# sailab-code/GNN_tf_2.x

Measured on AMD Instinct MI355X. Metric: node-state-updates/sec (nodes x iters / s), 1M-node synthetic graph, higher is better.
Workload: dtype f32; 1 GPU; synthetic randomGraph-recipe graph, N=1000000 nodes, E=9999690 arcs, state_dim=64, net_state 135->128->128->64 selu+BN, net_output 67->2 softmax+BN, max_iter=30, threshold=0 (all iterations run); the loop-invariant label aggregates (GNN.py:259, :263; 0.2 ms) are kept between Loops until the labels change, see cold_aggregates_ms_per_step; parallelism=single GPU, tile_form=one wave per 32-node tile (k_fused)

## Files before the change

gnn_tf_2.x_amd/csrc/gnn_build.hip:

```cpp
#include <hipcub/hipcub.hpp>
#include <string.h>

#include <algorithm>
#include <chrono>
#include <new>
#include <vector>

#include "gnn_common.h"
#include "gnn_fused.h"

namespace {

inline unsigned cdiv(int64_t a, int64_t b) { return (unsigned)((a + b - 1) / b); }

__global__ void k_keys(int64_t e, const int32_t *src, const int32_t *dst, unsigned long long *key, int32_t *id, int32_t *indeg)
{
    const int64_t a = (int64_t)blockIdx.x * blockDim.x + threadIdx.x;
    if (a >= e) return;
    key[a] = ((unsigned long long)(uint32_t)dst[a] << 32) | (uint32_t)src[a];
    id[a] = (int32_t)a;
    atomicAdd(indeg + dst[a], 1);
}

__global__ void k_values(int64_t e, const int32_t *dst, const int32_t *indeg, int mode, float *w)
// ... 217 lines not shown
                };
                for (int r = start[g]; r < start[g + 1]; ++r) {
                    if (ip[r + 1] == ip[r]) put(GNN_GP_NOROW | GNN_GP_ROW_END | (uint32_t)r, 0.0f);
                    for (int32_t e = ip[r]; e < ip[r + 1]; ++e) {
                        if (adj_src[e] < 0 || adj_src[e] >= (1 << 23))
                            return gnn_fail(GNN_ERR_UNSUPPORTED, "adj_src[%d]=%d does not fit a gather-program source word", e, adj_src[e]);
                        put((uint32_t)adj_src[e] << 8 | (e + 1 == ip[r + 1] ? GNN_GP_ROW_END : 0u) | (uint32_t)r, adj_w[e]);
                    }
                }
                while (s < 16 * nb) put(GNN_GP_NOROW, 0.0f);
            }
        }
        batch += nb;
    }
    *n_batches = batch;
    return GNN_OK;
}

int gnn_gather_program_ensure(const gnn_graph *g)
{
    gnn_graph_shared *sh = g->sh;
    if (sh->gp_tried) return GNN_OK;
    sh->gp_tried = true;
    const int64_t tiles = g->n_rows / 32;
    if (tiles == 0) return GNN_OK;
    int dev_before = -1;
    if (hipGetDevice(&dev_before) != hipSuccess || hipSetDevice(g->device) != hipSuccess) { (void)hipGetLastError(); return GNN_OK; }
    const auto t0 = std::chrono::steady_clock::now();
    int32_t *d_hdr = nullptr, *d_ent = nullptr;
    int64_t batches = 0;
    bool ok = false;
    try {
        std::vector<int32_t> indptr((size_t)tiles * 32 + 1), hdr((size_t)tiles * 2), src, ent;
        std::vector<float> w;
        ok = hipMemcpy(indptr.data(), sh->indptr, sizeof(int32_t) * indptr.size(), hipMemcpyDeviceToHost) == hipSuccess;
        const size_t E = ok ? (size_t)indptr.back() : 0;
        src.resize(E); w.resize(E);
        ok = ok && (E == 0 || (hipMemcpy(src.data(), sh->adj_src, sizeof(int32_t) * E, hipMemcpyDeviceToHost) == hipSuccess &&
                               hipMemcpy(w.data(), sh->adj_w, sizeof(float) * E, hipMemcpyDeviceToHost) == hipSuccess));
        for (size_t e = 0; ok && e < E; ++e) ok = src[e] >= 0 && src[e] < (1 << 23);
        ok = ok && gnn_gather_program_build(tiles * 32, indptr.data(), src.data(), w.data(), hdr.data(), nullptr, &batches) == GNN_OK;
        if (ok) {
            ent.resize((size_t)batches * 128);
            ok = gnn_gather_program_build(tiles * 32, indptr.data(), src.data(), w.data(), nullptr, ent.data(), &batches) == GNN_OK;
        }
        ok = ok && gnn_dev_malloc((void **)&d_hdr, sizeof(int32_t) * hdr.size()) == hipSuccess &&
             gnn_dev_malloc((void **)&d_ent, sizeof(int32_t) * ent.size()) == hipSuccess &&
             hipMemcpy(d_hdr, hdr.data(), sizeof(int32_t) * hdr.size(), hipMemcpyHostToDevice) == hipSuccess &&
             hipMemcpy(d_ent, ent.data(), sizeof(int32_t) * ent.size(), hipMemcpyHostToDevice) == hipSuccess;
    } catch (const std::bad_alloc &) { ok = false; }
    if (ok) {
        sh->gp_hdr = d_hdr; sh->gp_ent = d_ent; sh->gp_tiles = tiles; sh->gp_batches = batches;
        sh->gp_build_ms = std::chrono::duration<float, std::milli>(std::chrono::steady_clock::now() - t0).count();
    } else {
        (void)hipFree(d_hdr); (void)hipFree(d_ent);
        (void)hipGetLastError();
    }
    (void)hipSetDevice(dev_before);
    return GNN_OK;
}

extern "C" int gnn_graph_gather_program_info(const gnn_graph *g, int64_t *tiles, int64_t *batches, int64_t *bytes, float *build_ms)
{
    ARGCHK(g, "graph is NULL");
    const gnn_graph_shared *sh = g->sh;
    const bool have = sh->gp_ent != nullptr;
    if (tiles) *tiles = have ? sh->gp_tiles : 0;
    if (batches) *batches = have ? sh->gp_batches : 0;
    if (bytes) *bytes = have ? sh->gp_tiles * 8 + sh->gp_batches * 512 : 0;
    if (build_ms) *build_ms = have ? sh->gp_build_ms : 0.0f;
    return GNN_OK;
}
```

gnn_tf_2.x_amd/csrc/gnn_common.h:

```cpp
#pragma once
#include <hip/hip_runtime.h>
#include <stdint.h>
#include <string>
#include <vector>

#include "gnn_hip.h"
#include "gnn_fused.h"

int gnn_fail(int code, const char *fmt, ...);

hipError_t gnn_dev_malloc(void **p, size_t bytes);
bool gnn_poison_enabled();

inline hipError_t gnn_raise_dynamic_lds(const void *const *kernels, int n, size_t bytes, bool (&raised)[64])
{
    int dev = 0;
    hipError_t e = hipGetDevice(&dev);
    if (e != hipSuccess) return e;
    const bool listed = dev >= 0 && dev < 64;
    if (listed && raised[dev]) return hipSuccess;
    for (int i = 0; i < n && e == hipSuccess; ++i) e = hipFuncSetAttribute(kernels[i], hipFuncAttributeMaxDynamicSharedMemorySize, (int)bytes);
    if (listed && e == hipSuccess) raised[dev] = true;
    return e;
}
// ... 109 lines not shown
    const int c0 = __hip_atomic_load(w, __ATOMIC_RELAXED, __HIP_MEMORY_SCOPE_AGENT);
    const int c1 = __hip_atomic_load(w + 1, __ATOMIC_RELAXED, __HIP_MEMORY_SCOPE_AGENT);
    const int c2 = __hip_atomic_load(w + 2, __ATOMIC_RELAXED, __HIP_MEMORY_SCOPE_AGENT);
    if (moved && c0 == 0) atomicOr(w, 1);
    if (robust && c1 == 0) atomicOr(w + 1, 1);
    if (border && c2 == 0) atomicOr(w + 2, 1);
}

struct gnn_graph_shared {
    int refs = 1;
    int32_t *indptr = nullptr, *adj_src = nullptr, *masked_rows = nullptr;
    float *adj_w = nullptr, *arc_w = nullptr, *arc_labels = nullptr;
    uint8_t *mask = nullptr;
    int max_degree = 0;
    int32_t *src_indptr = nullptr, *src_dst = nullptr;
    float *src_w = nullptr;
    int32_t *arc_id = nullptr;
    float *arc_labels_orig = nullptr;
    int32_t *full_indptr = nullptr, *full_src = nullptr;
    float *full_w = nullptr;
    int64_t full_rows = 0;
    int32_t *gp_hdr = nullptr, *gp_ent = nullptr;
    int64_t gp_tiles = 0, gp_batches = 0;
    bool gp_tried = false;
    float gp_build_ms = 0.0f;
};

struct gnn_graph {
    int device = 0;
    int64_t N = 0, N_global = 0, row_begin = 0, own_off = 0, n_rows = 0, E = 0, n_masked = 0;
    int NL = 0, AL = 0;
    int halo_world = 0, halo_rank = 0;
    int64_t halo_block = 0, halo_count = 0;
    int32_t *halo_send = nullptr;
    bool halo_send_owned = true;
    int64_t nodes_rows = 0;
    gnn_graph_shared *sh = nullptr;
    float *nodes = nullptr;
    int base_NL = 0;
    float *arc_labels_own = nullptr, *arc_labels_orig_own = nullptr;
    int base_AL = 0;
    uint64_t label_version = 1;
    hipEvent_t ready = nullptr;
};

inline const float *gnn_graph_arc_labels(const gnn_graph *g) { return g->arc_labels_own ? g->arc_labels_own : g->sh->arc_labels; }
// ... 152 lines not shown
```

gnn_tf_2.x_amd/csrc/gnn_fused.h:

```cpp
#pragma once
#include <hip/hip_runtime.h>
#include <stdint.h>

constexpr int GNN_FUSED_MAXL = 3;
constexpr int GNN_FUSED_WAVES = 8;
constexpr int GNN_FUSED_THREADS = 64 * GNN_FUSED_WAVES;
#define GNN_F16_EX 4
#define GNN_F16_LIMIT 65504.0f
#define GNN_GP_ROW_MASK 31u
#define GNN_GP_ROW_END 32u
#define GNN_GP_NOROW 0xfffffe00u
constexpr int GNN_ACTL_FROM_ARGS = -1;

struct GnnFusedArgs {
    int64_t n_rows, row_begin;
    const int32_t *indptr, *adj_src;
    const float *adj_w;
    const float *inv;
    const float *state_cur;
    float *state_nxt;
    int64_t state_bytes;
    int Ds, NLc, AL, IW, in_s, c_aggs, KP, lpr, lpr_log2, vec, kk0;
    const float *Wp[GNN_FUSED_MAXL];
    const float *bias[GNN_FUSED_MAXL];
    const float *bn_scale, *bn_shift;
    float thr;
    const int *gate;
    int *flag_out;
    int world;
    int certify;
    int *tile_ctr;
    int wstride;
    int stagger;
    const int *Ws[GNN_FUSED_MAXL];
    int chunks0;
    int pieces;
    float bsc[GNN_FUSED_MAXL], usc[GNN_FUSED_MAXL];
    const int *Ws_base;
    int ws_bytes, ws_off[GNN_FUSED_MAXL];
    int tile_base;
    int full_tiles;
    int variant;
    const float *agg_in;
    const int32_t *gp_hdr, *gp_ent;
    int gp_tiles;
    int threads;
    int single_ticket;
    unsigned long long *stamps;
    int lds_floats;
    int act_last;
};

struct GnnSmallCtl {
    float *state0, *state1;
    const float *init;
    int *kfinal;
    int *flags;
    int *host_result;
    float *xs;
    int DP;
    int rnd;
    const float *Wraw[GNN_FUSED_MAXL];
    int din[GNN_FUSED_MAXL], dout[GNN_FUSED_MAXL];
    int KP16;
    int *zero_words;
    int n_words;
    int max_iter;
    float *out;
// ... 88 lines not shown
```

gnn_tf_2.x_amd/csrc/gnn_fused.hip:

```cpp
#include <stdio.h>
#include <stdlib.h>
#include <string.h>

#include <algorithm>
#include <cmath>
#include <vector>

#include "gnn_engine.h"
#include "gnn_fused.h"

namespace {

constexpr int MAXL = GNN_FUSED_MAXL;
constexpr int K_GROUP = 12;
constexpr int K_SLACK = 8;

constexpr int GNN_FUSED_VARIANT_DEFAULT = 1;
constexpr int GNN_FUSED_SPREAD_DEFAULT = 8;
constexpr int GNN_FUSED_SPREAD_SMALL_DEFAULT = 6;
#ifndef GNN_GATHER_FORM_DEFAULT
#define GNN_GATHER_FORM_DEFAULT 2
#endif
constexpr int S_SLACK = 2;

// ... 380 lines not shown
    static const int stagger_env = getenv("GNN_FUSED_STAGGER") ? atoi(getenv("GNN_FUSED_STAGGER")) : GNN_FUSED_SPREAD_DEFAULT;
    stagger_rounds = stagger_env;
#endif
    a.stagger = n_tiles >= (size_t)4 * GNN_FUSED_WAVES * grid ? stagger_rounds : (n_tiles > (size_t)GNN_FUSED_WAVES * grid ? GNN_FUSED_SPREAD_SMALL_DEFAULT : 0);
#ifdef GNN_DIAG
    static const int stagger_small = getenv("GNN_FUSED_STAGGER_SMALL") ? atoi(getenv("GNN_FUSED_STAGGER_SMALL")) : 0;
    const bool small_grid = n_tiles > (size_t)GNN_FUSED_WAVES * grid && n_tiles < (size_t)4 * GNN_FUSED_WAVES * grid;
    if (small_grid && stagger_small > 0) { a.stagger = stagger_small; a.variant |= 4; }
    static const int spread_small = getenv("GNN_FUSED_SPREAD_SMALL") ? atoi(getenv("GNN_FUSED_SPREAD_SMALL")) : -1;
    if (small_grid && spread_small >= 0) a.stagger = spread_small;
#endif
    a.single_ticket = n_tiles <= (size_t)GNN_FUSED_WAVES * grid ? 1 : 0;
    f.grid = grid;
    f.lds = lds_bytes(p);
    if (f.kernel == GNN_BODY_PAIR) {
        const int64_t n_tiles64 = (int64_t)n_tiles;
        a.KP = pair_xs(p);
        a.full_tiles = 1;
        f.grid = (unsigned)std::min<int64_t>((int64_t)n_cu, (n_tiles64 + 3) / 4);
        a.stagger = n_tiles64 >= (int64_t)4 * 4 * f.grid ? stagger_rounds : (n_tiles64 > (int64_t)4 * f.grid ? GNN_FUSED_SPREAD_SMALL_DEFAULT : 0);
        f.lds = pair_lds_bytes(p);
    } else if (f.kernel == GNN_BODY_FULL_TILE) {
        a.full_tiles = 1;
        if (f.program) { a.gp_hdr = g->sh->gp_hdr; a.gp_ent = g->sh->gp_ent; a.gp_tiles = (int)g->sh->gp_tiles; }
    }
    a.lds_floats = gnn_poison_enabled() ? (int)(f.lds / sizeof(float)) : 0;
}

static int decide_persistent(gnn_loop *l, LoopForm &f, const SmallForm &sf)
{
    const gnn_graph *g = l->g;
    const FusedPlan &p = f.plan;
    GnnFusedArgs &a = f.args;
    fill_args(l, p, false, a);
    a.state_cur = l->state[0];
    a.state_nxt = l->state[1] + (size_t)l->own_off * l->Ds;
    GnnSmallCtl &c = f.ctl;
    c.state0 = l->state[0]; c.state1 = l->state[1];
    c.init = l->D ? l->state_init : g->nodes + (size_t)g->own_off * g->NL;
    c.kfinal = l->kfinal_dev;
    c.host_result = l->kfinal_host;
    bool tile16 = sf.tile == 16;
    f.small_wide = sf.wide;
    if (tile16) f.s0 = sf.steps; else f.kk_small = sf.steps;
#ifdef GNN_DIAG
    static const int tile_env = getenv("GNN_SMALL_TILE") ? atoi(getenv("GNN_SMALL_TILE")) : 0;
    if (tile_env == 32 && !sf.wide) {
// ... 53 lines not shown
    a.lds_floats = gnn_poison_enabled() ? (int)(f.lds / sizeof(float)) : 0;
    return GNN_OK;
}

int gnn_loop_decide_form(gnn_loop *l)
{
    LoopForm &f = l->form;
    f = LoopForm{};
    if (l->impl_req < 1) return GNN_OK;
    HIPCHK(hipSetDevice(l->device));
    if (!gnn_fused_supported(l, f.plan)) return GNN_OK;
    if (l->device < 0 || l->device >= 64) return gnn_fail(GNN_ERR_ARG, "device %d out of range", l->device);
    const gnn_graph *g = l->g;
    const FusedPlan &p = f.plan;
    const int n_cu = device_cus(l->device);
    const int64_t n_tiles = (g->n_rows + 31) / 32;
    f.split = l->impl_req == 2;
    f.pieces = l->pieces == 2 ? 2 : 3;
    const bool pair = f.split && !l->slice_mode && pair_covers(p, l->Ds) && pair_lds_bytes(p) <= 160 * 1024 &&
                      (l->tile_form ? l->tile_form == 2 : n_tiles <= (int64_t)4 * n_cu);
    f.kernel = pair ? GNN_BODY_PAIR : (l->Ds == 64 && p.NTL == 2 ? GNN_BODY_FULL_TILE : GNN_BODY_GENERIC);
    if (f.kernel == GNN_BODY_FULL_TILE && !l->slice_mode && (l->gather_form ? l->gather_form : GNN_GATHER_FORM_DEFAULT) == 2 &&
        gnn_gather_program_ensure(g) == GNN_OK)
        f.program = g->sh->gp_ent != nullptr;
    const SmallForm sf = small_form(l->st, p, g->n_rows);
    const bool persistent = l->world == 1 && !l->small_disabled && !l->profiling && sf.tile != 0;
    f.path = persistent ? GNN_PATH_PERSISTENT : GNN_PATH_BODIES;
    if (!l->inv) HIPCHK(gnn_dev_malloc((void **)&l->inv, inv_floats(l) * sizeof(float)));
    if (persistent) return decide_persistent(l, f, sf);
    decide_bodies(l, f, n_cu);
    return GNN_OK;
}

static bool launch_body(const LoopForm &f, const GnnFusedArgs &a, hipStream_t st)
{
    const FusedPlan &p = f.plan;
    if (p.act_last != p.act) {
        if (f.kernel == GNN_BODY_PAIR || p.layers < 2) return false;
        if (f.split) return p.layers == 2 ? gnn_fused_launch_ms2(p.act, p.NT, p.NTL, a, f.grid, f.lds, st) : gnn_fused_launch_ms3(p.act, p.NT, p.NTL, a, f.grid, f.lds, st);
        return p.layers == 2 ? gnn_fused_launch_ml2(p.act, p.NT, p.NTL, a, f.grid, f.lds, st) : gnn_fused_launch_ml3(p.act, p.NT, p.NTL, a, f.grid, f.lds, st);
    }
    if (f.kernel == GNN_BODY_PAIR)
        return p.layers == 2 ? gnn_fused_launch_p2(p.act, a, f.grid, f.lds, st) : gnn_fused_launch_p3(p.act, a, f.grid, f.lds, st);
    if (f.split) {
        if (p.layers == 1) return gnn_fused_launch_s1(p.act, p.NT, p.NTL, a, f.grid, f.lds, st);
        if (p.layers == 2) return gnn_fused_launch_s2(p.act, p.NT, p.NTL, a, f.grid, f.lds, st);
        return gnn_fused_launch_s3(p.act, p.NT, p.NTL, a, f.grid, f.lds, st);
// ... 86 lines not shown
```

gnn_tf_2.x_amd/csrc/gnn_fused_kernel.h:

```cpp
#pragma once
#include <utility>

#include "gnn_common.h"
#include "gnn_fused.h"

typedef float f32x16 __attribute__((ext_vector_type(16)));

namespace gnn_fused_dev {

#define GNN_GLOBAL __attribute__((address_space(1)))
template <class T>
__device__ __forceinline__ const GNN_GLOBAL T *gptr(const T *p) { return (const GNN_GLOBAL T *)p; }
template <class T>
__device__ __forceinline__ GNN_GLOBAL T *gptr_w(T *p) { return (GNN_GLOBAL T *)p; }
typedef float v4f __attribute__((ext_vector_type(4)));
typedef float v2f __attribute__((ext_vector_type(2)));
typedef int v4i_ __attribute__((ext_vector_type(4)));
__device__ __forceinline__ v4f gload4(const float *p) { return *(const GNN_GLOBAL v4f *)p; }
#ifndef GNN_STORE_AUX
#define GNN_STORE_AUX 2
#endif
__device__ __forceinline__ void gstore_row4(float *base, int64_t off, v4f v)
{
#if GNN_STORE_AUX == 0
// ... 504 lines not shown
        GNN_S0_LOAD(wa, xa, c + 1)
        GNN_S0_MFMA(wb, pb, xa, pa, false, c + 1 < n_chunks)
        GNN_S0_LOAD(wb, xb, c + 2)
        if (c + 1 < n_chunks) GNN_S0_MFMA(wa, pa, xb, pb, false, c + 2 < n_chunks)
    }
#undef GNN_S0_LOAD
#undef GNN_S0_MFMA
}

template <int NO, bool AL16>
__device__ __forceinline__ void layer0_split(const float *xr, __amdgpu_buffer_rsrc_t wrs, int voff, int soff, int n_chunks, f32x16 (&acc)[NO],
                                             const float *bias_lds, int half)
{
    float mx = 0.0f;
    layer0_split<NO, AL16, 3>(xr, wrs, voff, soff, n_chunks, acc, bias_lds, half, mx);
}

template <int NI, int NO, int ACT, int PC = 3>
__device__ __forceinline__ void layer_split_from_regs(f32x16 (&hin)[NI], const float *bias_lds, int half, f32x16 (&acc)[NO],
                                                      __amdgpu_buffer_rsrc_t wrs, int voff, int soff, float us, float &mx)
{
    using TM = SplitTerms<PC>;
    constexpr int TPU = NO >= 2 ? 2 : 1, UPC = NO / TPU, CH = 2 * NI, U = CH * UPC;
    constexpr int DEPTH = (NI + NO >= 8) ? 1 : 3;
    constexpr int NM = TM::N * NO, NTASK = 12;
    v4i w[U][TPU][PC];
    int bp[2][PC][4];
    WStream ws(soff);
#define GNN_S1_LOAD(UU)                                                                             \
    _Pragma("unroll") for (int t = 0; t < TPU; ++t)                                                 \
        _Pragma("unroll") for (int pc = 0; pc < PC; ++pc) w[UU][t][pc] = ws.next(wrs, voff);
#define GNN_S1_H(C, I) hin[(C) >> 1][8 * ((C) & 1) + (I)]
#define GNN_S1_E(C, I)                                                                              \
    if constexpr (ACT == GNN_ACT_SELU) {                                                            \
        constexpr float AL2_ = 1.6732632423543772f * 1.44269504088896341f;                          \
        const float v_ = PC == 2 ? GNN_S1_H(C, I) * us : GNN_S1_H(C, I);                            \
        GNN_S1_H(C, I) = v_ > 0.0f ? v_ : __builtin_fmaf(__builtin_amdgcn_exp2f(v_), AL2_, -AL2_);  \
    } else GNN_S1_H(C, I) = act_fast<ACT>(PC == 2 ? GNN_S1_H(C, I) * us : GNN_S1_H(C, I));
#define GNN_S1_S(C, J, DST)                                                                         \
    if constexpr (PC == 2) { float mz_ = 0.0f; split_pair_f16(GNN_S1_H(C, 2 * (J)), GNN_S1_H(C, 2 * (J) + 1), DST[0][J], DST[1][J], mz_); }   \
    else split_pair(GNN_S1_H(C, 2 * (J)), GNN_S1_H(C, 2 * (J) + 1), DST[0][J], DST[1][J], DST[PC - 1][J]);
#pragma unroll
    for (int u = 0; u < DEPTH && u < U; ++u) { GNN_S1_LOAD(u) }
    {
#pragma unroll
        for (int i = 0; i < 8; ++i) { GNN_S1_E(0, i) }
#pragma unroll
// ... 319 lines not shown
    if (t & GNN_GP_ROW_END) {
        float *xr = xo + __umul24(t & GNN_GP_ROW_MASK, (unsigned)KP);
        if constexpr (AL16) *reinterpret_cast<v4f *>(xr) = v4f{acc01.x, acc01.y, acc23.x, acc23.y};
        else { xr[0] = acc01.x; xr[1] = acc01.y; xr[2] = acc23.x; xr[3] = acc23.y; }
        acc01 = v2f{0.f, 0.f}; acc23 = v2f{0.f, 0.f};
    }
}
template <bool AL16, int GB, int... J>
__device__ __forceinline__ void prog_batch(int words, float my_w, __amdgpu_buffer_rsrc_t rsrc, int voff0, float (&w)[GB], v4f (&x)[GB],
                                           std::integer_sequence<int, J...>)
{
    ((w[J] = row_bcast_f<J>(my_w),
      x[J] = __builtin_bit_cast(v4f, __builtin_amdgcn_raw_buffer_load_b128(rsrc, (row_bcast_i<J>(words) & ~0xff) | voff0, 0, 0))), ...);
}
template <bool AL16, int GB, int... J>
__device__ __forceinline__ void prog_consume_all(int words, const float (&w)[GB], const v4f (&x)[GB], v2f &acc01, v2f &acc23, float *xo, int KP,
                                                 std::integer_sequence<int, J...>)
{
    (prog_consume<AL16, J>(words, w[J], x[J], acc01, acc23, xo, KP), ...);
}
typedef int v2i __attribute__((ext_vector_type(2)));
__device__ __forceinline__ v2i prog_header_request(const GnnFusedArgs &a, int tile)
{
    v2i h = {0, 0};
    if (tile < a.gp_tiles) h = *reinterpret_cast<const GNN_GLOBAL v2i *>(gptr(a.gp_hdr) + 2 * (int64_t)tile);
    return h;
}
__device__ __forceinline__ v2i prog_entry(const GnnFusedArgs &a, int b, int lane)
{
    return *reinterpret_cast<const GNN_GLOBAL v2i *>(gptr(a.gp_ent) + ((int64_t)b * 64 + lane) * 2);
}
template <bool AL16>
__device__ __forceinline__ void load_tile_prog64(const GnnFusedArgs &a, float *X, int64_t i0, int lane, int KP, int c_aggs, int first, int nb, v2i ent)
{
    constexpr int GB = 16;
    const int gl = lane & 15;
    TileOwn64<AL16> own;
    own.request(a, i0, lane);
    v2f acc01 = {0.f, 0.f}, acc23 = {0.f, 0.f};
    const __amdgpu_buffer_rsrc_t rsrc = __builtin_amdgcn_make_buffer_rsrc(const_cast<float *>(a.state_cur), 0, (int)a.state_bytes, 0x00020000);
    const int voff0 = gl * 16;
    float *xo = X + c_aggs + gl * 4;
    for (int b = 0; b < nb; ++b) {
        float w[GB];
        v4f x[GB];
        const int words = ent.x;
        prog_batch<AL16, GB>(words, __int_as_float(ent.y), rsrc, voff0, w, x, std::make_integer_sequence<int, GB>{});
        if (b + 1 < nb) ent = prog_entry(a, first + b + 1, lane);
        prog_consume_all<AL16, GB>(words, w, x, acc01, acc23, xo, KP, std::make_integer_sequence<int, GB>{});
    }
    own.write(a, X, i0, lane, KP, c_aggs);
}

template <bool AL16>
__device__ __forceinline__ void load_tile_given64(const GnnFusedArgs &a, float *X, int64_t i0, int lane, int KP, int c_aggs)
{
    constexpr int Ds = 64;
    v4f own[8], agg[8];
    {
        const float *src = a.state_cur + (a.row_begin + i0) * Ds + lane * 4;
        const float *sag = a.agg_in + i0 * Ds + lane * 4;
#pragma unroll
        for (int u = 0; u < 8; ++u) {
            own[u] = gload4(src + u * 256);
            agg[u] = gload4(sag + u * 256);
        }
    }
    float lab[4];
    const int IW = a.IW, nlab = 32 * IW;
    {
        const float *src = a.inv + i0 * IW;
#pragma unroll
        for (int u = 0; u < 4; ++u) lab[u] = (lane + 64 * u < nlab) ? gload1(src + lane + 64 * u) : 0.0f;
    }
#pragma unroll
    for (int u = 0; u < 8; ++u) {
// ... 69 lines not shown
        for (int u = 0; u < 16; ++u) {
            const float d = half ? o[u] : (nw[u] - o[u]);
            const float dd = d * d;
            s_ = s_ + dd;
        }
    }
    const float root = sqrtf(s_);
    const float nrm = shfl_f(root, (lane & 31) + 32);
    const float rhs = a.thr * nrm;
    const int moved = (half == 0) && (root > rhs);
    if (__any(moved) && lane == 0) gnn_flag_raise(a.flag_out);
    float *dst = a.state_nxt + i0 * Ds + lane;
    const float *xs = X + c_aggs + lane;
#pragma unroll
    for (int i = 0; i < 32; i += 8) {
        float v[8];
#pragma unroll
        for (int u = 0; u < 8; ++u) v[u] = xs[(i + u) * KP];
#pragma unroll
        for (int u = 0; u < 8; ++u) gstore_row1(dst + (i + u) * Ds, v[u]);
    }
}

__device__ __forceinline__ void finish_fast64_aligned(const GnnFusedArgs &a, float *X, f32x16 (&out)[2], int64_t i0, int lane, int KP, int c_aggs,
                                                      const GnnFlagPeek &peek)
{
    const int half = lane >> 5;
    float *xrow = X + (lane & 31) * KP;
    float d2 = 0.0f, o2 = 0.0f;
#pragma unroll
    for (int jt = 0; jt < 2; ++jt)
#pragma unroll
        for (int q = 0; q < 4; ++q) {
            const int f0 = 32 * jt + 8 * q + 4 * half;
            const v4f o = *reinterpret_cast<const v4f *>(xrow + f0);
            const v4f nw = {out[jt][4 * q], out[jt][4 * q + 1], out[jt][4 * q + 2], out[jt][4 * q + 3]};
            *reinterpret_cast<v4f *>(xrow + c_aggs + f0) = nw;
            const v4f d = nw - o;
            d2 = __builtin_fmaf(d.x, d.x, d2); d2 = __builtin_fmaf(d.y, d.y, d2); d2 = __builtin_fmaf(d.z, d.z, d2); d2 = __builtin_fmaf(d.w, d.w, d2);
            o2 = __builtin_fmaf(o.x, o.x, o2); o2 = __builtin_fmaf(o.y, o.y, o2); o2 = __builtin_fmaf(o.z, o.z, o2); o2 = __builtin_fmaf(o.w, o.w, o2);
        }
    d2 = d2 + shfl_f(d2, lane ^ 32);
    o2 = o2 + shfl_f(o2, lane ^ 32);
    const float root = sqrtf(d2), nrm = sqrtf(o2);
    {
        const float rhs = a.thr * nrm, band = GNN_BAND_ABS * nrm + GNN_BAND_REL * rhs;
        const bool am = __any(root > rhs), ar = __any(root > rhs + band), ab = __any(gnn_gate_borderline(root, rhs, band));
        if (lane == 0) gnn_flag_raise_peeked(a.flag_out, peek, am, ar, ab);
    }
    __builtin_amdgcn_fence(__ATOMIC_ACQ_REL, "wavefront");
    const int64_t dst = i0 * 64 + lane * 4;
    const float *xs = X + (lane >> 4) * KP + c_aggs + (lane & 15) * 4;
    v4f v[8];
#pragma unroll
    for (int u = 0; u < 8; ++u) v[u] = *reinterpret_cast<const v4f *>(xs + 4 * u * KP);
#pragma unroll
    for (int u = 0; u < 8; ++u) gstore_row4(a.state_nxt, dst + 256 * u, v[u]);
}

__device__ __forceinline__ void check_store_fast64_partial(const GnnFusedArgs &a, float *X, int64_t i0, int lane, int KP, int c_aggs, int nvalid)
{
    constexpr int Ds = 64;
    const int half = lane >> 5;
    const float *xo = X + (lane & 31) * KP, *xn = xo + c_aggs;
    float s_ = 0.0f;
#pragma unroll
    for (int f = 0; f < Ds; f += 16) {
        float o[16], nw[16];
#pragma unroll
        for (int u = 0; u < 16; ++u) { o[u] = xo[f + u]; nw[u] = xn[f + u]; }
// ... 102 lines not shown
    int tile = w_launch + a.tile_base, next_tile = w_launch + W_launch + a.tile_base;
    int ip_first_raw = 0;
    v2i hdr_first_raw = {0, 0};
    if constexpr (PROG) hdr_first_raw = prog_header_request(a, tile);
    else ip_first_raw = tile_rowptr_request(a, tile, lane);
    float *ep = lds + (size_t)GNN_FUSED_WAVES * 32 * KP + 32 + GNN_FUSED_WAVES * 36;
    for (int t = threadIdx.x; t < 3 * 32 * NTL; t += blockDim.x) {
        const int which = t / (32 * NTL), f = t - which * 32 * NTL;
        ep[t] = which == 0 ? a.bias[LAYERS - 1][f] * (SPLIT ? a.bsc[LAYERS - 1] : 1.0f) : (a.bn_scale ? (which == 1 ? a.bn_scale[f] : a.bn_shift[f]) : 0.0f);
    }
    float *hb = ep + 3 * 32 * NTL;
    if constexpr (SPLIT && LAYERS > 1)
        for (int t = threadIdx.x; t < (LAYERS - 1) * 32 * NT; t += blockDim.x)
            hb[t] = a.bias[t / (32 * NT)][t % (32 * NT)] * (ACT == GNN_ACT_SELU ? 1.44269504088896341f : 1.0f) * a.bsc[t / (32 * NT)];
    __syncthreads();
    if (a.stagger > 0) {
        int rounds = 0;
        if (a.variant & 4) rounds = wave >= GNN_FUSED_WAVES / 2 ? a.stagger : 0;
        else rounds = (int)((((unsigned)blockIdx.x * GNN_FUSED_WAVES + (unsigned)wave) * 0x9E3779B1u) >> 16) % (unsigned)(a.stagger + 1);
        for (int i = 0; i < rounds; ++i) __builtin_amdgcn_s_sleep(127);
    }
    int ip_cur = 0, src_cur = 0;
    float w_cur = 0.0f;
    int hdr_first = 0, hdr_nb = 0;
    v2i ent_cur = {0, 0};
    if constexpr (PROG) {
        hdr_first = __builtin_amdgcn_readfirstlane(hdr_first_raw.x); hdr_nb = __builtin_amdgcn_readfirstlane(hdr_first_raw.y);
        if (hdr_nb > 0) ent_cur = prog_entry(a, hdr_first, lane);
    } else {
        ip_cur = tile_rowptr_clamp(a, tile, lane, ip_first_raw);
        if (FULL || Ds == 64) tile_first_ids(a, ip_cur, lane, src_cur, w_cur);
    }
    if constexpr (FULL) zero_pad_columns(a, X, lane, KP);
  for (;;) {
    const int64_t i0 = (int64_t)tile * 32;
    if (i0 >= a.n_rows) break;
    const int nvalid = (int)((a0.n_rows - i0) < 32 ? (a0.n_rows - i0) : 32);
    GnnFusedArgs a = a0;
    asm volatile("" : "+s"(a.Wp[0]), "+s"(a.Wp[1]), "+s"(a.Wp[2]), "+s"(a.bias[0]), "+s"(a.bias[1]), "+s"(a.bias[2]));
    asm volatile("" : "+s"(a.bn_scale), "+s"(a.bn_shift), "+s"(a.state_cur), "+s"(a.state_nxt), "+s"(a.inv), "+s"(a.adj_src), "+s"(a.adj_w));
#ifndef GNN_DIAG
#define GNN_STAMP(slot) do { } while (0)
#else
    unsigned long long *stamp = a.stamps ? a.stamps + ((size_t)tile << 3) : nullptr;
#define GNN_STAMP(slot)                                                                      \
    do {                                                                                     \
        if (stamp) {                                                                         \
            __builtin_amdgcn_sched_barrier(0);                                               \
            const unsigned long long t_ = __builtin_amdgcn_s_memtime();                      \
            if (lane == 0) stamp[slot] = t_;                                                 \
            __builtin_amdgcn_sched_barrier(0);                                               \
        }                                                                                    \
    } while (0)
#endif
    GNN_STAMP(0);

    int *ipt = reinterpret_cast<int *>(lds + (size_t)GNN_FUSED_WAVES * 32 * KP + 32) + wave * 36;
    int ip_next_raw = 0;
    v2i hdr_next_raw = {0, 0};
    if constexpr (PROG) hdr_next_raw = prog_header_request(a, next_tile);
    else {
        if (lane <= 32) ipt[lane] = ip_cur;
        ip_next_raw = tile_rowptr_request(a, next_tile, lane);
    }
    const bool fast64 = FULL || ((Ds == 64) && (nvalid == 32) && !a.agg_in);
    if (a.variant & 1) __builtin_amdgcn_s_setprio(3);
    if constexpr (FULL && GIVEN) load_tile_given64<SPLIT>(a, X, i0, lane, KP, c_aggs);
    else if constexpr (PROG) {
        if (hdr_nb > 0) load_tile_prog64<SPLIT>(a, X, i0, lane, KP, c_aggs, hdr_first, hdr_nb, ent_cur);
        else {
            const int ip = tile_rowptr_clamp(a, tile, lane, tile_rowptr_request(a, tile, lane));
            if (lane <= 32) ipt[lane] = ip;
            tile_first_ids(a, ip, lane, src_cur, w_cur);
            load_tile_fast64<SPLIT, true>(a, X, ipt, i0, lane, KP, c_aggs, src_cur, w_cur);
        }
    }
    else if constexpr (FULL) load_tile_fast64<SPLIT, true>(a, X, ipt, i0, lane, KP, c_aggs, src_cur, w_cur);
    else {
        if (fast64) load_tile_fast64<SPLIT>(a, X, ipt, i0, lane, KP, c_aggs, src_cur, w_cur);
        else load_tile_generic(a, X, ipt, i0, lane, nvalid, KP, c_aggs);
    }
    if (a.variant & 1) __builtin_amdgcn_s_setprio(0);
    __builtin_amdgcn_fence(__ATOMIC_ACQ_REL, "wavefront");
    GNN_STAMP(2);

    const int half = lane >> 5;
    const float *xb = X + (lane & 31) * KP + half;
    f32x16 out[NTL];
    float mx = 0.0f;
    if constexpr (SPLIT) {
        const __amdgpu_buffer_rsrc_t wrs = __builtin_amdgcn_make_buffer_rsrc(const_cast<int *>(a.Ws_base), 0, a.ws_bytes, 0x00020000);
        const int wv = lane * 16;
        const float *xr = X + (lane & 31) * KP + 8 * half;
        if constexpr (LAYERS == 1) {
            layer0_split<NTL, false, PC>(xr, wrs, wv, a.ws_off[0], a.chunks0, out, ep, half, mx);
        } else {
            f32x16 h1[NT];
            if constexpr (FULL) layer0_split<NT, true, PC>(xr, wrs, wv, a.ws_off[0], a.chunks0, h1, hb, half, mx);
            else {
// ... 14 lines not shown
        }
    } else if constexpr (LAYERS == 1) {
        zero_acc<NTL>(out);
        layer_from_lds<NTL>(xb, a.Wp[0] + (size_t)lane * NTL, a.kk0, out, a.wstride);
    } else {
        f32x16 h1[NT];
        zero_acc<NT>(h1);
        layer_from_lds<NT>(xb, a.Wp[0] + (size_t)lane * NT, a.kk0, h1, a.wstride);
        GNN_STAMP(3);
        GNN_STAMP(4);
        if constexpr (LAYERS == 2) {
            zero_acc<NTL>(out);
            layer_from_regs<NT, NTL, ACT>(h1, a.bias[0], half, out, a.Wp[1] + (size_t)lane * NTL, a.wstride);
        } else {
            f32x16 h2[NT];
            zero_acc<NT>(h2);
            layer_from_regs<NT, NT, ACT>(h1, a.bias[0], half, h2, a.Wp[1] + (size_t)lane * NT, a.wstride);
            zero_acc<NTL>(out);
            layer_from_regs<NT, NTL, ACT>(h2, a.bias[1], half, out, a.Wp[2] + (size_t)lane * NTL, a.wstride);
        }
    }
    __builtin_amdgcn_fence(__ATOMIC_ACQ_REL, "wavefront");
    GNN_STAMP(5);
    int next2_tile = 0x3fffffff;
    if (third_round) {
        if (lane == 0) next2_tile = atomicAdd(a0.tile_ctr, 1) + 2 * W_launch;
    }
    int ip_next = 0, src_next = 0;
    float w_next = 0.0f;
    int hdr_first_next = 0, hdr_nb_next = 0;
    v2i ent_next = {0, 0};
    if constexpr (PROG) {
        hdr_first_next = __builtin_amdgcn_readfirstlane(hdr_next_raw.x); hdr_nb_next = __builtin_amdgcn_readfirstlane(hdr_next_raw.y);
        if (hdr_nb_next > 0) ent_next = prog_entry(a, hdr_first_next, lane);
    } else {
        ip_next = tile_rowptr_clamp(a, next_tile, lane, ip_next_raw);
        if (FULL || Ds == 64) tile_first_ids(a, ip_next, lane, src_next, w_next);
    }
    if constexpr (SPLIT && PC == 2) gnn_flag_raise_range(a.flag_out, mx);
    GnnFlagPeek peek = {0, 0, 0};
    if (SPLIT && NTL == 2 && lane == 0) peek = gnn_flag_peek(a.flag_out);
    bool finished = false;
    if constexpr (SPLIT && NTL == 2) {
        if (fast64) {
#pragma unroll
            for (int jt = 0; jt < NTL; ++jt) {
                if (a.bn_scale) tile_epilogue_last<ACTL, true, true, true, true>(a.act_last, out[jt], ep, ep + 32 * NTL, ep + 64 * NTL, jt, half, 1 << 30, a.usc[LAYERS - 1]);
                else tile_epilogue_last<ACTL, false, true, true, true>(a.act_last, out[jt], ep, nullptr, nullptr, jt, half, 1 << 30, a.usc[LAYERS - 1]);
            }
            GNN_STAMP(6);
            if (nvalid == 32) finish_fast64_aligned(a, X, out, i0, lane, KP, c_aggs, peek);
            else finish_fast64_partial(a, X, out, i0, lane, KP, c_aggs, nvalid);
            finished = true;
        }
    }
    if (!(FULL && SPLIT && NTL == 2) && !finished) {
#pragma unroll
        for (int jt = 0; jt < NTL; ++jt) {
            const float us = SPLIT ? a.usc[LAYERS - 1] : 1.0f;
            if (a.bn_scale) tile_epilogue_last<ACTL, true, SPLIT, true, SPLIT>(a.act_last, out[jt], ep, ep + 32 * NTL, ep + 64 * NTL, jt, half, 1 << 30, us);
            else tile_epilogue_last<ACTL, false, SPLIT, true, SPLIT>(a.act_last, out[jt], ep, nullptr, nullptr, jt, half, 1 << 30, us);
            float *x = X + (lane & 31) * KP + c_aggs;
#pragma unroll
            for (int r = 0; r < 16; ++r) {
                const int f = 32 * jt + (r & 3) + 8 * (r >> 2) + 4 * half;
                if (f < Ds) x[f] = out[jt][r];
            }
        }
        __builtin_amdgcn_fence(__ATOMIC_ACQ_REL, "wavefront");
        GNN_STAMP(6);
        if constexpr (FULL) {
            if (nvalid == 32) check_store_fast64(a, X, i0, lane, KP, c_aggs);
            else check_store_fast64_partial(a, X, i0, lane, KP, c_aggs, nvalid);
        } else {
            if (fast64) check_store_fast64(a, X, i0, lane, KP, c_aggs);
            else check_store_generic(a, X, i0, lane, nvalid, KP, c_aggs);
        }
    }
    GNN_STAMP(7);
#undef GNN_STAMP
    __builtin_amdgcn_fence(__ATOMIC_ACQ_REL, "wavefront");
    tile = next_tile;
    next_tile = __builtin_amdgcn_readfirstlane(next2_tile) + a0.tile_base;
    ip_cur = ip_next; src_cur = src_next; w_cur = w_next;
    hdr_first = hdr_first_next; hdr_nb = hdr_nb_next; ent_cur = ent_next;
  }
}

template <int LAYERS, int NT, int NTL, int ACT, bool SPLIT, int ACTL, bool FULL, bool GIVEN = false, int PC = 3, bool PROG = false>
inline void launch_one_pc(const GnnFusedArgs &a, unsigned grid, size_t lds_bytes, hipStream_t st)
{
    if constexpr (FULL && !GIVEN && !PROG) {
        if (a.gp_tiles > 0) { launch_one_pc<LAYERS, NT, NTL, ACT, SPLIT, ACTL, FULL, GIVEN, PC, true>(a, grid, lds_bytes, st); return; }
    }
    static bool lds_raised[64] = {false};
    (void)gnn_raise_dynamic_lds(reinterpret_cast<const void *>(&k_fused<LAYERS, NT, NTL, ACT, SPLIT, FULL, GIVEN, PC, PROG, ACTL>), 160 * 1024, lds_raised);
    hipLaunchKernelGGL((k_fused<LAYERS, NT, NTL, ACT, SPLIT, FULL, GIVEN, PC, PROG, ACTL>), grid, a.threads ? a.threads : GNN_FUSED_THREADS, lds_bytes, st, a);
}
template <int LAYERS, int NT, int NTL, int ACT, bool SPLIT, int ACTL, bool FULL, bool GIVEN = false>
inline void launch_one(const GnnFusedArgs &a, unsigned grid, size_t lds_bytes, hipStream_t st)
{
    if (SPLIT && a.pieces == 2) launch_one_pc<LAYERS, NT, NTL, ACT, SPLIT, ACTL, FULL, GIVEN, 2>(a, grid, lds_bytes, st);
    else launch_one_pc<LAYERS, NT, NTL, ACT, SPLIT, ACTL, FULL, GIVEN, 3>(a, grid, lds_bytes, st);
}

template <int LAYERS, int NT, int NTL, int ACT, bool SPLIT, int ACTL>
// ... 56 lines not shown
```

Measured before the change: 1.763 billion node-state-updates/s.

## Prefetch first gather-program batch of next tile during epilogue; cover partial last tile

Issues the buffer loads for the next tile's first gather batch, along with its second entry, before the current tile's epilogue and store, so neighbour-row fetch latency overlaps with compute. The gather program now also covers the trailing partial tile through extra header fields, which removes the CSR fallback path inside the program kernel. It adds register pressure from 16 prefetched v4f values held across the epilogue, reorders the flag raise and the tile-counter atomic, and adds a depth knob for the wide split path.

```diff
diff --git a/gnn_tf_2.x_amd/csrc/gnn_build.hip b/gnn_tf_2.x_amd/csrc/gnn_build.hip
--- a/gnn_tf_2.x_amd/csrc/gnn_build.hip
+++ b/gnn_tf_2.x_amd/csrc/gnn_build.hip
@@ -263,27 +263,33 @@
     gnn_graph_shared *sh = g->sh;
     if (sh->gp_tried) return GNN_OK;
     sh->gp_tried = true;
-    const int64_t tiles = g->n_rows / 32;
+    const int64_t tiles = g->n_rows / 32, rem = g->n_rows % 32;
     if (tiles == 0) return GNN_OK;
     int dev_before = -1;
     if (hipGetDevice(&dev_before) != hipSuccess || hipSetDevice(g->device) != hipSuccess) { (void)hipGetLastError(); return GNN_OK; }
     const auto t0 = std::chrono::steady_clock::now();
     int32_t *d_hdr = nullptr, *d_ent = nullptr;
-    int64_t batches = 0;
+    int64_t batches = 0, last_batches = 0;
+    int32_t last_hdr[2] = {0, 0};
     bool ok = false;
     try {
-        std::vector<int32_t> indptr((size_t)tiles * 32 + 1), hdr((size_t)tiles * 2), src, ent;
+        std::vector<int32_t> indptr((size_t)g->n_rows + 1), hdr((size_t)tiles * 2), src, ent;
         std::vector<float> w;
         ok = hipMemcpy(indptr.data(), sh->indptr, sizeof(int32_t) * indptr.size(), hipMemcpyDeviceToHost) == hipSuccess;
         const size_t E = ok ? (size_t)indptr.back() : 0;
+        if (rem) indptr.resize((size_t)(tiles + 1) * 32 + 1, indptr.back());
         src.resize(E); w.resize(E);
         ok = ok && (E == 0 || (hipMemcpy(src.data(), sh->adj_src, sizeof(int32_t) * E, hipMemcpyDeviceToHost) == hipSuccess &&
                                hipMemcpy(w.data(), sh->adj_w, sizeof(float) * E, hipMemcpyDeviceToHost) == hipSuccess));
         for (size_t e = 0; ok && e < E; ++e) ok = src[e] >= 0 && src[e] < (1 << 23);
+        const int32_t *last_ip = indptr.data() + tiles * 32;
         ok = ok && gnn_gather_program_build(tiles * 32, indptr.data(), src.data(), w.data(), hdr.data(), nullptr, &batches) == GNN_OK;
+        if (ok && rem) ok = gnn_gather_program_build(32, last_ip, src.data(), w.data(), last_hdr, nullptr, &last_batches) == GNN_OK;
+        ok = ok && batches + last_batches < ((int64_t)1 << 31) / 64;
         if (ok) {
-            ent.resize((size_t)batches * 128);
+            ent.resize((size_t)(batches + last_batches) * 128);
             ok = gnn_gather_program_build(tiles * 32, indptr.data(), src.data(), w.data(), nullptr, ent.data(), &batches) == GNN_OK;
+            if (ok && rem) ok = gnn_gather_program_build(32, last_ip, src.data(), w.data(), nullptr, ent.data() + (size_t)batches * 128, &last_batches) == GNN_OK;
         }
         ok = ok && gnn_dev_malloc((void **)&d_hdr, sizeof(int32_t) * hdr.size()) == hipSuccess &&
              gnn_dev_malloc((void **)&d_ent, sizeof(int32_t) * ent.size()) == hipSuccess &&
@@ -291,7 +297,8 @@
              hipMemcpy(d_ent, ent.data(), sizeof(int32_t) * ent.size(), hipMemcpyHostToDevice) == hipSuccess;
     } catch (const std::bad_alloc &) { ok = false; }
     if (ok) {
-        sh->gp_hdr = d_hdr; sh->gp_ent = d_ent; sh->gp_tiles = tiles; sh->gp_batches = batches;
+        sh->gp_hdr = d_hdr; sh->gp_ent = d_ent; sh->gp_tiles = tiles; sh->gp_batches = batches + last_batches;
+        sh->gp_rows = g->n_rows; sh->gp_last_first = (int32_t)batches; sh->gp_last_nb = (int32_t)last_batches;
         sh->gp_build_ms = std::chrono::duration<float, std::milli>(std::chrono::steady_clock::now() - t0).count();
     } else {
         (void)hipFree(d_hdr); (void)hipFree(d_ent);
diff --git a/gnn_tf_2.x_amd/csrc/gnn_common.h b/gnn_tf_2.x_amd/csrc/gnn_common.h
--- a/gnn_tf_2.x_amd/csrc/gnn_common.h
+++ b/gnn_tf_2.x_amd/csrc/gnn_common.h
@@ -155,6 +155,8 @@
     int64_t full_rows = 0;
     int32_t *gp_hdr = nullptr, *gp_ent = nullptr;
     int64_t gp_tiles = 0, gp_batches = 0;
+    int64_t gp_rows = 0;
+    int32_t gp_last_first = 0, gp_last_nb = 0;
     bool gp_tried = false;
     float gp_build_ms = 0.0f;
 };
diff --git a/gnn_tf_2.x_amd/csrc/gnn_fused.h b/gnn_tf_2.x_amd/csrc/gnn_fused.h
--- a/gnn_tf_2.x_amd/csrc/gnn_fused.h
+++ b/gnn_tf_2.x_amd/csrc/gnn_fused.h
@@ -43,7 +43,7 @@
     int variant;
     const float *agg_in;
     const int32_t *gp_hdr, *gp_ent;
-    int gp_tiles;
+    int gp_tiles, gp_last_first, gp_last_nb;
     int threads;
     int single_ticket;
     unsigned long long *stamps;
diff --git a/gnn_tf_2.x_amd/csrc/gnn_fused.hip b/gnn_tf_2.x_amd/csrc/gnn_fused.hip
--- a/gnn_tf_2.x_amd/csrc/gnn_fused.hip
+++ b/gnn_tf_2.x_amd/csrc/gnn_fused.hip
@@ -426,7 +426,10 @@
         f.lds = pair_lds_bytes(p);
     } else if (f.kernel == GNN_BODY_FULL_TILE) {
         a.full_tiles = 1;
-        if (f.program) { a.gp_hdr = g->sh->gp_hdr; a.gp_ent = g->sh->gp_ent; a.gp_tiles = (int)g->sh->gp_tiles; }
+        if (f.program) {
+            a.gp_hdr = g->sh->gp_hdr; a.gp_ent = g->sh->gp_ent; a.gp_tiles = (int)g->sh->gp_tiles;
+            a.gp_last_first = g->sh->gp_last_first; a.gp_last_nb = g->sh->gp_last_nb;
+        }
     }
     a.lds_floats = gnn_poison_enabled() ? (int)(f.lds / sizeof(float)) : 0;
 }
@@ -526,7 +529,7 @@
     f.kernel = pair ? GNN_BODY_PAIR : (l->Ds == 64 && p.NTL == 2 ? GNN_BODY_FULL_TILE : GNN_BODY_GENERIC);
     if (f.kernel == GNN_BODY_FULL_TILE && !l->slice_mode && (l->gather_form ? l->gather_form : GNN_GATHER_FORM_DEFAULT) == 2 &&
         gnn_gather_program_ensure(g) == GNN_OK)
-        f.program = g->sh->gp_ent != nullptr;
+        f.program = g->sh->gp_ent != nullptr && g->sh->gp_rows == g->n_rows;
     const SmallForm sf = small_form(l->st, p, g->n_rows);
     const bool persistent = l->world == 1 && !l->small_disabled && !l->profiling && sf.tile != 0;
     f.path = persistent ? GNN_PATH_PERSISTENT : GNN_PATH_BODIES;
diff --git a/gnn_tf_2.x_amd/csrc/gnn_fused_kernel.h b/gnn_tf_2.x_amd/csrc/gnn_fused_kernel.h
--- a/gnn_tf_2.x_amd/csrc/gnn_fused_kernel.h
+++ b/gnn_tf_2.x_amd/csrc/gnn_fused_kernel.h
@@ -550,7 +550,10 @@
 {
     using TM = SplitTerms<PC>;
     constexpr int TPU = NO >= 2 ? 2 : 1, UPC = NO / TPU, CH = 2 * NI, U = CH * UPC;
-    constexpr int DEPTH = (NI + NO >= 8) ? 1 : 3;
+#ifndef GNN_S1_DEPTH_WIDE
+#define GNN_S1_DEPTH_WIDE 1
+#endif
+    constexpr int DEPTH = (NI + NO >= 8) ? (PC == 2 ? GNN_S1_DEPTH_WIDE : 1) : 3;
     constexpr int NM = TM::N * NO, NTASK = 12;
     v4i w[U][TPU][PC];
     int bp[2][PC][4];
@@ -916,7 +919,7 @@
 typedef int v2i __attribute__((ext_vector_type(2)));
 __device__ __forceinline__ v2i prog_header_request(const GnnFusedArgs &a, int tile)
 {
-    v2i h = {0, 0};
+    v2i h = {a.gp_last_first, tile == a.gp_tiles ? a.gp_last_nb : 0};
     if (tile < a.gp_tiles) h = *reinterpret_cast<const GNN_GLOBAL v2i *>(gptr(a.gp_hdr) + 2 * (int64_t)tile);
     return h;
 }
@@ -946,6 +949,59 @@
     own.write(a, X, i0, lane, KP, c_aggs);
 }
 
+#ifndef GNN_FIRST_BATCH_AHEAD
+#define GNN_FIRST_BATCH_AHEAD 1
+#endif
+template <int GB, int... J>
+__device__ __forceinline__ void prog_rows_request(int words, __amdgpu_buffer_rsrc_t rsrc, int voff0, v4f (&x)[GB], std::integer_sequence<int, J...>)
+{
+    ((x[J] = __builtin_bit_cast(v4f, __builtin_amdgcn_raw_buffer_load_b128(rsrc, (row_bcast_i<J>(words) & ~0xff) | voff0, 0, 0))), ...);
+}
+template <bool AL16, int GB, int... J>
+__device__ __forceinline__ void prog_consume_first(v2i ent, const v4f (&x)[GB], v2f &acc01, v2f &acc23, float *xo, int KP, std::integer_sequence<int, J...>)
+{
+    (prog_consume<AL16, J>(ent.x, row_bcast_f<J>(__int_as_float(ent.y)), x[J], acc01, acc23, xo, KP), ...);
+}
+__device__ __forceinline__ void prog_first_batch_request(const GnnFusedArgs &a, int first, int nb, v2i ent0, int lane, v4f (&x0)[16], v2i &ent1)
+{
+    const __amdgpu_buffer_rsrc_t rsrc = __builtin_amdgcn_make_buffer_rsrc(const_cast<float *>(a.state_cur), 0, (int)a.state_bytes, 0x00020000);
+    if (nb > 1) ent1 = prog_entry(a, first + 1, lane);
+    __builtin_amdgcn_sched_barrier(0);
+    prog_rows_request<16>(ent0.x, rsrc, (lane & 15) * 16, x0, std::make_integer_sequence<int, 16>{});
+}
+template <bool AL16>
+__device__ __forceinline__ void load_tile_prog64_ahead(const GnnFusedArgs &a, float *X, int64_t i0, int lane, int KP, int c_aggs, int first, int nb,
+                                                       v2i ent0, const v4f (&x0)[16], v2i ent, v2i hdr_next_raw, int &first_next, int &nb_next,
+                                                       v2i &ent_next)
+{
+    constexpr int GB = 16;
+    const int gl = lane & 15;
+    TileOwn64<AL16> own;
+    own.request(a, i0, lane);
+    v2f acc01 = {0.f, 0.f}, acc23 = {0.f, 0.f};
+    const __amdgpu_buffer_rsrc_t rsrc = __builtin_amdgcn_make_buffer_rsrc(const_cast<float *>(a.state_cur), 0, (int)a.state_bytes, 0x00020000);
+    const int voff0 = gl * 16;
+    float *xo = X + c_aggs + gl * 4;
+    auto request_next = [&]() {
+        first_next = __builtin_amdgcn_readfirstlane(hdr_next_raw.x); nb_next = __builtin_amdgcn_readfirstlane(hdr_next_raw.y);
+        ent = v2i{(int)GNN_GP_NOROW, 0};
+        if (nb_next > 0) ent = prog_entry(a, first_next, lane);
+    };
+    if (nb <= 1) request_next();
+    prog_consume_first<AL16, GB>(ent0, x0, acc01, acc23, xo, KP, std::make_integer_sequence<int, GB>{});
+    for (int b = 1; b < nb; ++b) {
+        float w[GB];
+        v4f x[GB];
+        const int words = ent.x;
+        prog_batch<AL16, GB>(words, __int_as_float(ent.y), rsrc, voff0, w, x, std::make_integer_sequence<int, GB>{});
+        if (b + 1 < nb) ent = prog_entry(a, first + b + 1, lane);
+        else request_next();
+        prog_consume_all<AL16, GB>(words, w, x, acc01, acc23, xo, KP, std::make_integer_sequence<int, GB>{});
+    }
+    ent_next = ent;
+    own.write(a, X, i0, lane, KP, c_aggs);
+}
+
 template <bool AL16>
 __device__ __forceinline__ void load_tile_given64(const GnnFusedArgs &a, float *X, int64_t i0, int lane, int KP, int c_aggs)
 {
@@ -1061,8 +1117,9 @@
     }
 }
 
+template <bool LATE = false>
 __device__ __forceinline__ void finish_fast64_aligned(const GnnFusedArgs &a, float *X, f32x16 (&out)[2], int64_t i0, int lane, int KP, int c_aggs,
-                                                      const GnnFlagPeek &peek)
+                                                      GnnFlagPeek peek)
 {
     const int half = lane >> 5;
     float *xrow = X + (lane & 31) * KP;
@@ -1085,6 +1142,7 @@
     {
         const float rhs = a.thr * nrm, band = GNN_BAND_ABS * nrm + GNN_BAND_REL * rhs;
         const bool am = __any(root > rhs), ar = __any(root > rhs + band), ab = __any(gnn_gate_borderline(root, rhs, band));
+        if constexpr (LATE) asm volatile("" : "+v"(peek.c0), "+v"(peek.c1), "+v"(peek.c2));
         if (lane == 0) gnn_flag_raise_peeked(a.flag_out, peek, am, ar, ab);
     }
     __builtin_amdgcn_fence(__ATOMIC_ACQ_REL, "wavefront");
@@ -1233,11 +1291,14 @@
     }
     int ip_cur = 0, src_cur = 0;
     float w_cur = 0.0f;
+    constexpr bool AHEAD = PROG && GNN_FIRST_BATCH_AHEAD && !(SPLIT && PC == 3 && NT == 4);
     int hdr_first = 0, hdr_nb = 0;
-    v2i ent_cur = {0, 0};
+    v2i ent_cur = {AHEAD ? (int)GNN_GP_NOROW : 0, 0}, ent_second = {0, 0};
+    v4f x_first[16];
     if constexpr (PROG) {
         hdr_first = __builtin_amdgcn_readfirstlane(hdr_first_raw.x); hdr_nb = __builtin_amdgcn_readfirstlane(hdr_first_raw.y);
         if (hdr_nb > 0) ent_cur = prog_entry(a, hdr_first, lane);
+        if constexpr (AHEAD) prog_first_batch_request(a, hdr_first, hdr_nb, ent_cur, lane, x_first, ent_second);
     } else {
         ip_cur = tile_rowptr_clamp(a, tile, lane, ip_first_raw);
         if (FULL || Ds == 64) tile_first_ids(a, ip_cur, lane, src_cur, w_cur);
@@ -1266,8 +1327,10 @@
 #endif
     GNN_STAMP(0);
 
-    int *ipt = reinterpret_cast<int *>(lds + (size_t)GNN_FUSED_WAVES * 32 * KP + 32) + wave * 36;
+    [[maybe_unused]] int *ipt = reinterpret_cast<int *>(lds + (size_t)GNN_FUSED_WAVES * 32 * KP + 32) + wave * 36;
     int ip_next_raw = 0;
+    int hdr_first_next = 0, hdr_nb_next = 0;
+    v2i ent_next = {0, 0};
     v2i hdr_next_raw = {0, 0};
     if constexpr (PROG) hdr_next_raw = prog_header_request(a, next_tile);
     else {
@@ -1277,15 +1340,9 @@
     const bool fast64 = FULL || ((Ds == 64) && (nvalid == 32) && !a.agg_in);
     if (a.variant & 1) __builtin_amdgcn_s_setprio(3);
     if constexpr (FULL && GIVEN) load_tile_given64<SPLIT>(a, X, i0, lane, KP, c_aggs);
-    else if constexpr (PROG) {
-        if (hdr_nb > 0) load_tile_prog64<SPLIT>(a, X, i0, lane, KP, c_aggs, hdr_first, hdr_nb, ent_cur);
-        else {
-            const int ip = tile_rowptr_clamp(a, tile, lane, tile_rowptr_request(a, tile, lane));
-            if (lane <= 32) ipt[lane] = ip;
-            tile_first_ids(a, ip, lane, src_cur, w_cur);
-            load_tile_fast64<SPLIT, true>(a, X, ipt, i0, lane, KP, c_aggs, src_cur, w_cur);
-        }
-    }
+    else if constexpr (AHEAD)
+        load_tile_prog64_ahead<SPLIT>(a, X, i0, lane, KP, c_aggs, hdr_first, hdr_nb, ent_cur, x_first, ent_second, hdr_next_raw, hdr_first_next, hdr_nb_next, ent_next);
+    else if constexpr (PROG) load_tile_prog64<SPLIT>(a, X, i0, lane, KP, c_aggs, hdr_first, hdr_nb, ent_cur);
     else if constexpr (FULL) load_tile_fast64<SPLIT, true>(a, X, ipt, i0, lane, KP, c_aggs, src_cur, w_cur);
     else {
         if (fast64) load_tile_fast64<SPLIT>(a, X, ipt, i0, lane, KP, c_aggs, src_cur, w_cur);
@@ -1346,24 +1403,32 @@
     }
     __builtin_amdgcn_fence(__ATOMIC_ACQ_REL, "wavefront");
     GNN_STAMP(5);
+    if constexpr (AHEAD && SPLIT && PC == 2) gnn_flag_raise_range(a.flag_out, mx);
     int next2_tile = 0x3fffffff;
     if (third_round) {
-        if (lane == 0) next2_tile = atomicAdd(a0.tile_ctr, 1) + 2 * W_launch;
+        int64_t ctr_off = 0;
+        if constexpr (AHEAD) asm volatile("" : "+v"(ctr_off));
+        if constexpr (AHEAD) { if (lane == 0) next2_tile = atomicAdd(a0.tile_ctr + ctr_off, 1); }
+        else if (lane == 0) next2_tile = atomicAdd(a0.tile_ctr, 1) + 2 * W_launch;
     }
     int ip_next = 0, src_next = 0;
     float w_next = 0.0f;
-    int hdr_first_next = 0, hdr_nb_next = 0;
-    v2i ent_next = {0, 0};
-    if constexpr (PROG) {
+    if constexpr (AHEAD) { }
+    else if constexpr (PROG) {
         hdr_first_next = __builtin_amdgcn_readfirstlane(hdr_next_raw.x); hdr_nb_next = __builtin_amdgcn_readfirstlane(hdr_next_raw.y);
         if (hdr_nb_next > 0) ent_next = prog_entry(a, hdr_first_next, lane);
     } else {
         ip_next = tile_rowptr_clamp(a, next_tile, lane, ip_next_raw);
         if (FULL || Ds == 64) tile_first_ids(a, ip_next, lane, src_next, w_next);
     }
-    if constexpr (SPLIT && PC == 2) gnn_flag_raise_range(a.flag_out, mx);
+    if constexpr (!AHEAD && SPLIT && PC == 2) gnn_flag_raise_range(a.flag_out, mx);
     GnnFlagPeek peek = {0, 0, 0};
     if (SPLIT && NTL == 2 && lane == 0) peek = gnn_flag_peek(a.flag_out);
+    if constexpr (AHEAD) {
+        __builtin_amdgcn_sched_barrier(0);
+        prog_first_batch_request(a, hdr_first_next, hdr_nb_next, ent_next, lane, x_first, ent_second);
+        __builtin_amdgcn_sched_barrier(0);
+    }
     bool finished = false;
     if constexpr (SPLIT && NTL == 2) {
         if (fast64) {
@@ -1373,7 +1438,7 @@
                 else tile_epilogue_last<ACTL, false, true, true, true>(a.act_last, out[jt], ep, nullptr, nullptr, jt, half, 1 << 30, a.usc[LAYERS - 1]);
             }
             GNN_STAMP(6);
-            if (nvalid == 32) finish_fast64_aligned(a, X, out, i0, lane, KP, c_aggs, peek);
+            if (nvalid == 32) finish_fast64_aligned<AHEAD>(a, X, out, i0, lane, KP, c_aggs, peek);
             else finish_fast64_partial(a, X, out, i0, lane, KP, c_aggs, nvalid);
             finished = true;
         }
@@ -1405,7 +1470,10 @@
 #undef GNN_STAMP
     __builtin_amdgcn_fence(__ATOMIC_ACQ_REL, "wavefront");
     tile = next_tile;
-    next_tile = __builtin_amdgcn_readfirstlane(next2_tile) + a0.tile_base;
+    if constexpr (AHEAD) {
+        asm volatile("" : "+v"(next2_tile));
+        next_tile = __builtin_amdgcn_readfirstlane(next2_tile) + (third_round ? 2 * W_launch : 0) + a0.tile_base;
+    } else next_tile = __builtin_amdgcn_readfirstlane(next2_tile) + a0.tile_base;
     ip_cur = ip_next; src_cur = src_next; w_cur = w_next;
     hdr_first = hdr_first_next; hdr_nb = hdr_nb_next; ent_cur = ent_next;
   }
```

Measured after the change: 1.788 billion node-state-updates/s (median of 6 runs). +1.4%, better.
